# okgarces/deep-successor-features-for-transfer

Hardware: AMD Instinct MI355X
Metric: env steps/sec (whole node), Reacher 8-task SF-DQN at 1/2/4/8 MI355X (higher is better)
Workload: dtype fp32; 1 GPU; reacher17-all-T8-B32 (Reacher-shape |s|=17 |a|=7 d=8, psi MLP 256x2, all heads updated per env step: main_sfdqn_torch.py path); heads_per_gpu=8, heads_total=8, global_batch=32, replay=host, parallelism=single

## Files before the change

deep-successor-features-for-transfer_amd/csrc/sfx.hip:

```cpp
#include <hip/hip_ext.h>
#include <hip/hip_runtime.h>
#include <dlfcn.h>
#include <rccl/rccl.h>

#include <cmath>
#include <cstdio>
#include <cstdlib>
#include <cstring>
#include <algorithm>
#include <atomic>
#include <chrono>
#include <deque>
#include <map>
#include <random>
#include <string>
#include <functional>
#include <tuple>
#include <utility>
#include <vector>

#include "sfx_kernels.h"
#include "sfx_gpiw.h"
#include "sfx_tsf.h"
#include "sfx_phi.h"
// ... 512 lines not shown
  A.npol = npol;
  A.guess = guess;
  A.flag = flag;
  A.flag_value = h->T;
  A.next_stride = next_stride;
  A.a = a;
  A.phi = phi;
  A.gamma = gamma;
  A.next = next;
  A.prev = skip ? prev : nullptr;
  A.skip = skip ? h->skip : nullptr;
  A.skipc = skip ? h->skipc : nullptr;
  launch(h, K_TDG, by, k_tdg, dim3(M, npol), dim3(256), h->G, A);
  LAUNCHCHK();
  return SFX_OK;
}

struct TdgSpec {
  int use_gpi = 1, guess = R_S1, next_stride = 0;
  const int64_t* a = nullptr;
  const float* gamma = nullptr;
  int64_t* next = nullptr;
  int* flag = nullptr;
  const int* xmax = nullptr;
  int poloff = 0;
  const int* xi_src = nullptr;
  int* xi_dst = nullptr;
  int xi_copy = 0, xi_n = 0;
  const int64_t* prev = nullptr;
  bool skip = false;
  const float* dz_scale = nullptr;
};

int tdg_variant(const sfx_handle* h) {
  if ((h->d & 3) != 0 || h->O > TDG_ROWS_O || h->A > 128) return 0;
  const long ta = (long)h->T * h->A;
  if (h->d <= 8 && 32 * ta <= 256 * 8) return 1;
  if (h->d <= 16 && 32 * ta <= 256 * 4) return 2;
  return 0;
}

bool can_fuse_tdg(const sfx_handle* h) { return tdg_variant(h) != 0; }

struct BwdExtra {
  int inc_step = 1;
  bool fuse_v0 = false;
  int vRole = R_V;
  const float* v_x = nullptr;
  const float* v_xn = nullptr;
  bool skip_fwd = false;
  const float* ax = nullptr;
  int aM = 0, a_noskip = 0;
  bool* skip_armed = nullptr;
  std::function<bool(int li, int tail_at, const BwdArgs& A, int ntile, double bytes)> ride;
};

bool can_fuse_v0(const sfx_handle* h, int vM) { return h->L[0].K <= KFUSE && vM * h->L[0].K <= VFUSE; }
bool can_fuse_ahead(const sfx_handle* h, int vM, int aM) {
  const int K = h->L[0].K;
  return can_fuse_v0(h, vM) && ((vM * K + 3) & ~3) + 2 * aM * K <= VFUSE && (2 * aM * K) % 4 == 0;
}

int run_bwd(sfx_handle* h, int head0, int nhead, int M, const float* x0, const float* phi, const float* r,
            float* losses, const TdgSpec& td, const BwdExtra& ex = BwdExtra()) {
  const bool fuse = can_fuse_tdg(h) && ((uintptr_t)phi & 15) == 0 &&
                    (!td.xmax || 32 * h->A <= 1024);
  if (!fuse && td.xi_dst) SFX_FAIL(SFX_E_STATE, "run_bwd: maxima re-initialisation needs the fused TD launch");
  const bool armed = td.skip && (fuse ? M <= 32 : true);
  if (!fuse)
    RC(run_tdg(h, head0, nhead, td.guess, M, td.use_gpi, td.a, phi, td.gamma, td.next, td.next_stride, td.flag,
               td.xmax, td.poloff, td.dz_scale, td.prev, armed));
  if (ex.skip_armed) *ex.skip_armed = armed;
  const int tail_at = fuse ? 1 : 0;
  const bool need_tail = losses || r || !fuse;
  BwdArgs A{};
  A.M = M;
  A.head0 = head0;
  A.nhead = nhead;
  A.xcd = nhead > 1 ? 1 : 0;
  A.mask = h->mask;
  A.hp = h->hp_psi;
  A.hpw = h->hp_w;
  A.x0 = x0;
  A.phi = phi;
  A.r = r;
  A.train_w = r != nullptr;
  A.losses = losses;
  A.inc_step = ex.inc_step;
  A.step_in_tail = fuse ? 0 : 1;
  A.tdg_use_gpi = td.use_gpi;
  A.tdg_guess = td.guess;
  A.tdg_next_stride = td.next_stride;
  A.tdg_a = td.a;
  A.tdg_gamma = td.gamma;
  A.tdg_next = td.next;
  A.tdg_xmax = td.xmax;
  A.tdg_poloff = td.poloff;
  A.flag = td.flag;
  A.flag_value = h->T;
  A.dz_scale = td.dz_scale;
  A.xi_copy = td.xi_copy;
  A.xi_n = td.xi_n;
  A.dxs = 1;
  if (armed) {
    A.skip = h->skip;
    A.skip_v0 = ex.skip_fwd ? 1 : 0;
    if (fuse) {
      A.tdg_prev = td.prev;
      A.skipc = h->skipc;
    }
  }
  auto dw_tiles = [&](int l) { return cdiv(h->L[l].N, 32) * cdiv(h->L[l].K, 64); };
  auto geo = [&](int l) {
    const LayerGeo& L = h->L[l];
    const int xOff = l == 0 ? -1 : h->actOff[l - 1], dzIn = l == 0 ? 0 : h->actOff[l - 1];
    return RoleGeo{L.N, L.K, L.wOff, L.bOff, L.actIn, xOff,  h->actOff[l], dzIn};
  };
  auto dx_bytes = [&](int l) {
    const LayerGeo& L = h->L[l];
    return 4.0 * ((double)L.N * L.K + (double)M * L.N + 2.0 * M * L.K);
  };
  auto dw_bytes = [&](int l) {
    const LayerGeo& L = h->L[l];
    return 24.0 * ((double)L.N * L.K + L.N) + 4.0 * ((double)M * L.N + (double)M * L.K);
  };
  auto grid_of = [&](int ntile) { return A.xcd ? dim3(8 * cdiv(nhead, 8) * ntile) : dim3(ntile, nhead); };
  const bool merge = h->bwd_merge && nhead > 1 && !ex.ride && h->NL >= 3 && M <= 32 && ex.fuse_v0 &&
                     can_fuse_v0(h, M + (ex.v_xn ? 1 : 0)) && h->L[1].N <= DX_SPLIT_N;
  int l = h->NL - 1;
  if (fuse) {
    A.tdg = 1;
    A.xi_src = td.xi_src;
    A.xi_dst = td.xi_dst;
    A.ra = geo(l);
    const int ktiles = cdiv(h->L[l].K, 16);
    const bool rows16 = M > 16 && M <= 32 && h->tdg_rows != 32 &&
                        (h->tdg_rows == 16 || (nhead > 1 && !ex.ride && nhead * 2 * ktiles <= h->ncu));
    const int ntd = cdiv(M, rows16 ? 16 : 32) * ktiles;
    A.na = ntd;
    dim3 grid = grid_of(ntd);
    if (A.inc_step) A.adam_wg = (int)grid.x++ + 1;
    const double tdg_bytes = 4.0 * nhead * M * ((td.use_gpi ? h->T : 1) * h->O + 2.0 * h->O + 2.0 * h->d + 4);
    const bool v1 = tdg_variant(h) == 1;
    launch(h, K_BWD, nhead * dx_bytes(l) + tdg_bytes,
           rows16 ? (v1 ? k_bwd_tdg<2, 4, 16> : k_bwd_tdg<4, 2, 16>) : (v1 ? k_bwd_tdg<2, 8> : k_bwd_tdg<4, 4>), grid,
           dim3(256), h->G, A);
    A.adam_wg = 0;
    A.tdg = 0;
    A.xi_src = nullptr;
    A.xi_dst = nullptr;
    --l;
  }
  auto issue = [&](int li, bool mg, double by) {
    const int ntile = A.na + A.nb + A.nc + A.nd + A.tail;
    if (ex.ride && nhead == 1 && ex.ride(li, tail_at, A, ntile, by)) return;
    launch(h, K_BWD, by, !mg ? (h->bf16 ? k_bwd<true> : k_bwd<false>) : (h->bf16 ? k_bwd_mg<true> : k_bwd_mg<false>),
           grid_of(ntile), dim3(256), h->G, A);
  };
  for (; l >= (merge ? 2 : 1); --l) {
    const int li = h->NL - 1 - l;
    const bool dw = l < h->NL - 1;
    A.ra = geo(l);
    const bool split = h->dxpart && h->L[l].N > DX_SPLIT_N && M <= 32 * cdiv(h->Mmax, 32) && nhead <= h->T;
    A.dxs = split ? cdiv(h->L[l].N, DX_SPLIT_N) : 1;
    A.na = cdiv(M, 32) * cdiv(h->L[l].K, 16) * A.dxs;
    if (split) {
      A.dxpart = h->dxpart;
      A.dxctr = h->dxctr;
    }
    if (dw) {
      A.rb = geo(l + 1);
      A.nb = dw_tiles(l + 1);
    }
    A.tail = li == tail_at && need_tail ? 1 : 0;
    issue(li, false, nhead * (dx_bytes(l) + (dw ? dw_bytes(l + 1) : 0.0)));
  }
  const int last = merge ? h->NL - 2 : h->NL - 1;
  A.na = 0;
  A.dxs = 1;
  A.rb = geo(1);
  A.nb = dw_tiles(1);
  A.rc = geo(0);
  A.nc = dw_tiles(0);
  A.tail = last == tail_at && need_tail ? 1 : 0;
  double by_last = nhead * (dw_bytes(1) + dw_bytes(0));
  if (merge) {
    A.nc = cdiv(h->L[0].N, 16);
    A.ra = geo(1);
    A.rd = geo(2);
    A.nd = dw_tiles(2);
    by_last += nhead * (dw_bytes(2) + dx_bytes(1) - 4.0 * M * h->L[1].K - 4.0 * M * h->L[0].N);
  }
  A.vM = M + (ex.v_xn ? 1 : 0);
  A.vOff = h->actOff[0];
  A.vRole = ex.vRole;
  A.act0 = h->L[0].actOut;
  A.v_x = ex.v_x;
  A.v_xn = ex.v_xn;
  A.a_noskip = ex.a_noskip;
  if (ex.fuse_v0) {
    A.fuse_v0 = 1;
    A.ax = ex.ax;
    A.aM = ex.ax ? ex.aM : 0;
  }
  issue(last, merge, by_last);
  LAUNCHCHK();
  return SFX_OK;
}

GpiArgs gpi_args(int role, int rowoff, int row0, const float* w, float* psi, float* q, int64_t* task, int64_t* next,
                 int64_t* sel, int select_task, int use_gpi, int M) {
  GpiArgs A{};
  A.M = M;
  A.role = role;
  A.row0 = row0;
  A.rowoff = rowoff;
  A.select_task = select_task;
  A.use_gpi = use_gpi;
  A.w = w;
  A.psi_out = psi;
  A.q_out = q;
  A.task_out = task;
  A.next_out = next;
  A.sel_out = sel;
  return A;
}

int run_gpi(sfx_handle* h, const GpiArgs& A) {
  launch(h, K_GPI, 4.0 * A.M * ((double)h->T * h->O * (A.psi_out ? 2 : 1) + h->d + (A.q_out ? h->T * h->A : 0)),
         k_gpi, dim3(A.M), dim3(256), h->G, A);
  LAUNCHCHK();
  return SFX_OK;
}

int run_ver(sfx_handle* h, int M, int npol, bool sel, int post, const GpiArgs& g, const int64_t* spec,
            bool post_host = false) {
  VerArgs V{};
  V.M = M;
  V.post = post;
  V.npol = npol;
  V.sel = sel ? 1 : 0;
  V.spec_stride = MMAX;
  V.spec_next = spec;
  V.flag = &h->dout->flag;
  V.g = g;
  const int TA = h->T * h->A;
  V.rows = TA >= 256 ? 1 : (256 / TA < M ? 256 / TA : M);
  const bool wide = wide_gpi(h) && npol > 1;
  const dim3 grid = wide ? dim3(M, cdiv(npol, WPC) + 1) : dim3(npol + 1, cdiv(M, V.rows));
  if (sel && h->pub_res && h->fold_publish) {
    V.pub = h->pub_res;
    V.pub_dctr = h->pub_dctr;
    V.done = &h->dout->done;
    V.nblocks = (int)(grid.x * grid.y);
    h->pub_folded = true;
  } else if (post_host) {
    V.h_sel = h->hout->sel;
    V.h_flag = &h->hout->flag;
    V.h_posted = &h->hout->posted;
    V.done = &h->dout->done;
    V.nblocks = (int)(grid.x * grid.y);
    h->hout_posted = true;
  }
  const double by = 4.0 * (double)M * npol * h->T * h->O + 4.0 * h->T * h->O;
  if (wide)
    launch(h, K_VER, by, SFX_WIDE(k_verw), grid, dim3(256), h->G, V);
  else
    launch(h, K_VER, by, k_ver, grid, dim3(256), h->G, V);
  LAUNCHCHK();
  return SFX_OK;
}

void after_update(sfx_handle* h, int t) {
  h->host_step[t] += 1;
  h->since_target[t] += 1;
}

int maybe_sync_target(sfx_handle* h, int t) {
  if (h->since_target[t] >= h->target_update_ev) {
    touch(h);
    HIPCHK(hipMemcpyAsync(h->target_of(t), h->online_cur(t), sizeof(float) * h->P, hipMemcpyDeviceToDevice,
                          h->stream));
    if (h->bf16)
      HIPCHK(hipMemcpyAsync(h->tg16_of(t), h->on16_cur(t), sizeof(__bf16) * h->P, hipMemcpyDeviceToDevice,
                            h->stream));
    h->since_target[t] = 0;
  }
  return SFX_OK;
}

void pack_head(const sfx_handle* h, const float* src, float* dst) {
  std::memset(dst, 0, sizeof(float) * h->P);
  size_t off = 0;
  for (const LayerGeo& L : h->L) {
    std::memcpy(dst + L.wOff, src + off, sizeof(float) * L.N * L.K);
    off += (size_t)L.N * L.K;
    std::memcpy(dst + L.bOff, src + off, sizeof(float) * L.N);
    off += L.N;
  }
}

void unpack_head(const sfx_handle* h, const float* src, float* dst) {
  size_t off = 0;
  for (const LayerGeo& L : h->L) {
    std::memcpy(dst + off, src + L.wOff, sizeof(float) * L.N * L.K);
    off += (size_t)L.N * L.K;
    std::memcpy(dst + off, src + L.bOff, sizeof(float) * L.N);
    off += L.N;
  }
}

bool valid_head(const sfx_handle* h, int t) { return h && t >= 0 && t < h->T; }
bool valid_w(const sfx_handle* h, int t) { return h && t >= 0 && t < h->Tg; }

__global__ void k_to_bf16(const float* __restrict__ src, __bf16* __restrict__ dst, long long n) {
  for (long long i = (long long)blockIdx.x * blockDim.x + threadIdx.x; i < n; i += (long long)gridDim.x * blockDim.x)
    dst[i] = (__bf16)src[i];
}

int refresh_bf16(sfx_handle* h, const float* src, __bf16* dst, long long n) {
  touch(h);
  hipLaunchKernelGGL(k_to_bf16, dim3((unsigned)std::min<long long>(1024, (n + 255) / 256)), dim3(256), 0, h->stream, src,
                     dst, n);
  LAUNCHCHK();
  return SFX_OK;
}

void free_all(sfx_handle* h) {
  clear_graphs(h);
  for (auto& r : h->prof_recs) {
    (void)hipEventDestroy(r.a);
    (void)hipEventDestroy(r.b);
  }
  for (hipEvent_t e : h->prof_pool) (void)hipEventDestroy(e);
  for (void* p : {(void*)h->online, (void*)h->target, (void*)h->am, (void*)h->av, (void*)h->w, (void*)h->wm,
                  (void*)h->wv, (void*)h->step, (void*)h->dcancel, (void*)h->adamc, (void*)h->act, (void*)h->dz, (void*)h->rowloss, (void*)h->spec_next, (void*)h->skip, (void*)h->skipc,
                  (void*)h->dout, (void*)h->dxpart, (void*)h->dxctr, (void*)h->qh, (void*)h->selk})
    if (p) (void)hipFree(p);
  if (h->hout) (void)hipHostFree(h->hout);
  if (h->xin) (void)hipHostFree(h->xin);
  if (h->ev_step) (void)hipEventDestroy(h->ev_step);
  if (h->on16) (void)hipFree(h->on16);
  if (h->tg16) (void)hipFree(h->tg16);
  if (h->host_ar_buf) (void)hipHostFree(h->host_ar_buf);
  for (int* p : {h->tsx, h->tsz})
    if (p) (void)hipFree(p);
  for (int* p : {h->xb[0], h->xb[1]})
    if (p) (void)hipFree(p);
  if (h->comm_rounds) (void)rccl().CommDestroy(h->comm_rounds);
  if (h->comm && h->comm_owned) (void)rccl().CommDestroy(h->comm);
  if (h->dstall) (void)hipFree(h->dstall);
  if (h->cap) (void)hipStreamDestroy(h->cap);
}

int auto_spec_rounds(int T_glob) { return T_glob >= 16 ? 3 : 2; }

// ... 1167 lines not shown
```

deep-successor-features-for-transfer_amd/csrc/sfx_kernels.h:

```cpp
#pragma once
#include <hip/hip_runtime.h>
#include <stdint.h>

#include <type_traits>

namespace sfx {

typedef float floatx4 __attribute__((ext_vector_type(4)));

constexpr int NLMAX = 8;
constexpr int MT = 32;
constexpr int QMAX = 8192;
constexpr int OMAX = 4096;
constexpr int DMAX = 256;
constexpr int MMAX = 1024;
constexpr int KFUSE = 64;
constexpr int GEMV_N = 512;
constexpr int GEMV_M = 4;
constexpr int DX_SPLIT_N = 256;
constexpr int VFUSE = 4096;
constexpr int TQF = 4096;

enum { ACT_NONE = 0, ACT_RELU = 1, ACT_TANH = 2 };
enum { R_S = 0, R_S1T = 1, R_S1 = 2, R_G = 3, R_A = 4, R_V = 5, R_V2 = 6, R_NS = 7, R_NS1T = 8, R_NS1 = 9, NROLE = 10 };
// ... 823 lines not shown
    return z < huber ? __fmul_rn(__fmul_rn(0.5f, z), z) : __fmul_rn(huber, __fsub_rn(z, __fmul_rn(0.5f, huber)));
  }
  return __fmul_rn(x, x);
}

__device__ __forceinline__ void tdg_skip_report(int* skip, unsigned long long* skipc, int pol, int T, bool differs,
                                                bool have_prev, int nrep) {
  int* word = skip + T + pol;
  const int old = __hip_atomic_fetch_add(word, differs ? 0x10001 : 1, __ATOMIC_RELAXED, __HIP_MEMORY_SCOPE_AGENT);
  if ((old & 0xFFFF) == nrep - 1) {
    const bool any = (old >> 16) != 0 || differs;
    skip[pol] = any ? 0 : 1;
    if (skipc && have_prev) {
      atomicAdd(skipc, 1ull);
      if (!any) atomicAdd(skipc + 1, 1ull);
    }
    __hip_atomic_store(word, 0, __ATOMIC_RELAXED, __HIP_MEMORY_SCOPE_AGENT);
  }
}

struct TdgArgs {
  int M, use_gpi, pol0, npol, guess, next_stride, flag_value, pad_;
  const int64_t* a;
  const float* phi;
  const float* gamma;
  int64_t* next;
  int* flag;
  const int* xmax;
  int poloff, pad2_;
  const float* dz_scale;
  const int64_t* prev;
  int* skip;
  unsigned long long* skipc;
};

__global__ __launch_bounds__(256) void k_tdg(Geo G, TdgArgs A) {
  PROBE_T(pt0);
  const int b = blockIdx.x, pol = A.pol0 + blockIdx.y, tid = threadIdx.x;
  const int T = G.T, Aa = G.A, d = G.d, O = G.O, M = A.M, NLm = G.lastOff;
  __shared__ float s_w[DMAX];
  __shared__ float s_q[QMAX];
  __shared__ float s_t[OMAX];
  __shared__ float s_m[256];
  __shared__ float s_sq[DMAX];
  __shared__ int s_next;
  const float* wrow = G.w + (long long)pol * G.dpad;
  for (int k = tid; k < d; k += 256) s_w[k] = wrow[k];
  if (A.flag && b == 0 && blockIdx.y == 0 && tid == 0) *A.flag = A.flag_value;
  const float* trow = G.actp(R_S1T, pol, NLm) + (size_t)b * O;
  for (int o = tid; o < O; o += 256) s_t[o] = trow[o];
  const int ab = (int)A.a[b];
  const bool aok = ab >= 0 && ab < Aa;
  float cval = 0.f, phik = 0.f;
  const float gam = A.gamma[b];
  if (tid < d) {
    phik = A.phi[(size_t)b * d + tid];
    if (aok) cval = G.actp(R_S, pol, NLm)[(size_t)b * O + ab * d + tid];
  }
  __syncthreads();
  if (A.xmax) {
    const int* xr = A.xmax + ((size_t)(A.poloff + pol) * M + b) * Aa;
    for (int a = tid; a < Aa; a += 256) s_m[a] = unsortable(xr[a]);
  } else {
    const int t0 = A.use_gpi ? 0 : pol, nt = A.use_gpi ? T : 1;
    const FDiv fA = fdiv(Aa);
    for (int idx = tid; idx < nt * Aa; idx += 256) {
      const int tq = idx / fA, t = t0 + tq, a = idx - tq * Aa;
      const float* p = G.actp(t < pol ? A.guess : R_S1, t, NLm) + (size_t)b * O + a * d;
      float q = 0.f;
#pragma unroll 8
      for (int k = 0; k < d; ++k) q = __builtin_fmaf(p[k], s_w[k], q);
      s_q[idx] = q;
    }
    __syncthreads();
    for (int a = tid; a < Aa; a += 256) {
      float mx = s_q[a];
      for (int t = 1; t < nt; ++t) mx = fmaxf(mx, s_q[t * Aa + a]);
      s_m[a] = mx;
    }
  }
  __syncthreads();
  if (tid == 0) {
    int am = 0;
    float qm = s_m[0];
    for (int a = 1; a < Aa; ++a)
      if (s_m[a] > qm) {
        qm = s_m[a];
        am = a;
      }
    s_next = am;
    SFX_CHK(b < A.next_stride || !A.next, b, A.next_stride, 0);
    if (A.next) A.next[(size_t)blockIdx.y * A.next_stride + b] = am;
    if (A.skip)
      tdg_skip_report(A.skip, A.skipc, pol, T, !A.prev || A.prev[(size_t)blockIdx.y * A.next_stride + b] != am,
                      A.prev != nullptr, M);
  }
  __syncthreads();
  const float norm = td_norm(G, M, O, A.dz_scale);
  float* grow = G.dzp(pol, NLm) + (size_t)b * O;
  const float* crow = G.actp(R_S, pol, NLm) + (size_t)b * O;
  const int an = s_next;
  for (int o = tid; o < O; o += 256) {
    float gv = 0.f;
    if (aok && o >= ab * d && o < ab * d + d) {
      const int k = o - ab * d;
      const float tg = __fadd_rn(A.phi[(size_t)b * d + k], __fmul_rn(gam, s_t[an * d + k]));
      gv = td_grad(G.huber, norm, __fsub_rn(crow[o], tg));
    }
    grow[o] = gv;
  }
  float dsq = 0.f;
  if (tid < d && aok) {
    const float diff = __fsub_rn(cval, __fadd_rn(phik, __fmul_rn(gam, s_t[an * d + tid])));
    dsq = td_loss(G.huber, diff);
    if (!__builtin_isfinite(diff) && G.nonfin) atomicOr(G.nonfin, 1);
  }
  if (tid < d) s_sq[tid] = dsq;
  __syncthreads();
  if (tid == 0) {
    float s = 0.f;
    for (int k = 0; k < d; ++k) s = __fadd_rn(s, s_sq[k]);
    SFX_CHK(pol >= 0 && pol < G.T && b < MMAX, pol, b, 0);
    G.rowloss[(long long)pol * MMAX + b] = s;
  }
  PROBE_REC(17, pt0);
}

struct RoleGeo {
  int N, K, wOff, bOff, actIn;
  int xOff;
  int dzOff;
  int dzIn;
};

struct BwdArgs {
  int M, na, nb, nc, tail, head0, train_w, inc_step;
  int xcd, nhead;
  int step_in_tail;
  int tdg, tdg_use_gpi, tdg_guess, tdg_next_stride, flag_value;
  int adam_wg;
  const int64_t* tdg_a;
  const float* tdg_gamma;
  int64_t* tdg_next;
  const int* tdg_xmax;
  int tdg_poloff, pad3_;
  int* flag;
  int fuse_v0, vM, vOff, act0;
  int vRole, dxs;
  unsigned long long mask;
  float* dxpart;
  unsigned* dxctr;
  RoleGeo ra, rb, rc;
  RoleGeo rd;
  int nd, pad5_;
  AdamHP hp, hpw;
  const float* x0;
  const float* phi;
  const float* r;
  float* losses;
  const float* v_x;
  const float* v_xn;
  const float* ax;
  int aM, a_noskip;
  const int* xi_src;
  int* xi_dst;
  int xi_copy, xi_n;
  const int64_t* tdg_prev;
  int* skip;
  unsigned long long* skipc;
  int skip_v0;
  const float* dz_scale;
};
static_assert(sizeof(BwdArgs) == 512, "BwdArgs: the kernel-argument layout of k_bwd* / k_bwd_tsf");

__device__ __forceinline__ const float* layer_input(const Geo& G, const BwdArgs& A, int head, int xOff) {
  return xOff < 0 ? A.x0 : G.actp(R_S, head, xOff);
}

constexpr int TDG_ROWS_O = 128;
template <int RT>
struct TdgSmem {
  float w[32], gam[RT], ph[RT * 16];
  int a[RT], n[RT];
  float q[RT * 64], m[RT * 128];
  float tt[RT * TDG_ROWS_O], tc[RT * TDG_ROWS_O];
  float dz[RT * TDG_ROWS_O];
};

template <int VMAX, int U, int RT>
__device__ int tdg_rows(const Geo& G, const BwdArgs& A, int pol, int m0, bool pub, TdgSmem<RT>& sm) {
  static_assert(RT == 32 || RT == 16, "row tile of the fused TD launch");
  constexpr int U4 = RT / 8;
  const int tid = threadIdx.x, T = G.T, Aa = G.A, d = G.d, O = G.O, NLm = G.lastOff, M = A.M;
  const int nb = M - m0 < RT ? M - m0 : RT;
  const bool xm = A.tdg_xmax != nullptr;
  const int t0 = A.tdg_use_gpi ? 0 : pol, nt = A.tdg_use_gpi ? T : 1, TA = nt * Aa, n = xm ? 0 : nb * TA, V = d >> 2;
  const int guess = A.tdg_guess;
  const FDiv fTA = fdiv(TA), fA = fdiv(Aa);
  float4 v[U][VMAX];
#pragma unroll
  for (int u = 0; u < U; ++u) {
    const int idx = tid + u * 256;
    const bool ok = idx < n;
    const int bl = idx / fTA, rem = idx - bl * TA, tq = rem / fA, t = t0 + tq, a = rem - tq * Aa;
    const float4* p = reinterpret_cast<const float4*>(G.actp(t < pol ? guess : R_S1, ok ? t : 0, NLm) +
                                                      (ok ? (size_t)(m0 + bl) * O + a * d : 0));
#pragma unroll
    for (int j = 0; j < VMAX; ++j) v[u][j] = (ok && j < V) ? p[j] : make_float4(0.f, 0.f, 0.f, 0.f);
  }
  const int n4 = (nb * O) >> 2;
  const float4* tg4 = reinterpret_cast<const float4*>(G.actp(R_S1T, pol, NLm) + (size_t)m0 * O);
  const float4* cu4 = reinterpret_cast<const float4*>(G.actp(R_S, pol, NLm) + (size_t)m0 * O);
  float4 tt[U4], tc[U4];
#pragma unroll
  for (int u = 0; u < U4; ++u) {
    const int i = tid + u * 256;
    tt[u] = i < n4 ? tg4[i] : make_float4(0.f, 0.f, 0.f, 0.f);
    tc[u] = i < n4 ? cu4[i] : make_float4(0.f, 0.f, 0.f, 0.f);
  }
  const int np4 = (nb * d) >> 2;
  const float4 ph = tid < np4 ? reinterpret_cast<const float4*>(A.phi + (size_t)m0 * d)[tid] : make_float4(0.f, 0.f, 0.f, 0.f);
  const float wk = tid < d ? G.w[(long long)pol * G.dpad + tid] : 0.f;
  const int ab_l = tid < nb ? (int)A.tdg_a[m0 + tid] : 0;
  const float gam_l = tid < nb ? A.tdg_gamma[m0 + tid] : 0.f;
  int xv[U4];
  if (xm) {
    const int* xr = A.tdg_xmax + ((size_t)(A.tdg_poloff + pol) * M + m0) * Aa;
#pragma unroll
    for (int u = 0; u < U4; ++u) xv[u] = tid + u * 256 < nb * Aa ? xr[tid + u * 256] : 0;
  }
  const int64_t* prev = A.tdg_prev ? A.tdg_prev + (size_t)(pol - A.head0) * A.tdg_next_stride + m0 : nullptr;
  const int64_t prev_l = prev && tid < nb ? prev[tid] : -1;
#pragma unroll
  for (int u = 0; u < U4; ++u) {
    const int i = tid + u * 256;
    if (i < n4) {
      reinterpret_cast<float4*>(sm.tt)[i] = tt[u];
      reinterpret_cast<float4*>(sm.tc)[i] = tc[u];
      reinterpret_cast<float4*>(sm.dz)[i] = make_float4(0.f, 0.f, 0.f, 0.f);
    }
  }
  if (tid < np4) reinterpret_cast<float4*>(sm.ph)[tid] = ph;
  if (tid < d) sm.w[tid] = wk;
  if (tid < nb) {
    sm.a[tid] = ab_l;
    sm.gam[tid] = gam_l;
  }
  __syncthreads();
  PROBE_AT(3);
  if (xm) {
#pragma unroll
    for (int u = 0; u < U4; ++u)
      if (tid + u * 256 < nb * Aa) sm.m[tid + u * 256] = unsortable(xv[u]);
  }
#pragma unroll
  for (int u = 0; u < U; ++u) {
    const int idx = tid + u * 256;
    float q = 0.f;
#pragma unroll
    for (int j = 0; j < VMAX; ++j) {
      if (j < V) {
        q = __builtin_fmaf(v[u][j].x, sm.w[4 * j], q);
        q = __builtin_fmaf(v[u][j].y, sm.w[4 * j + 1], q);
        q = __builtin_fmaf(v[u][j].z, sm.w[4 * j + 2], q);
        q = __builtin_fmaf(v[u][j].w, sm.w[4 * j + 3], q);
      }
    }
    if (idx < n) sm.q[idx] = q;
  }
  __syncthreads();
  PROBE_AT(5);
  for (int i = tid; i < (xm ? 0 : nb * Aa); i += 256) {
    const int bl = i / fA, a = i - bl * Aa;
    const float* qb = sm.q + bl * TA + a;
    float mx = qb[0];
    for (int t = 1; t < nt; ++t) mx = fmaxf(mx, qb[t * Aa]);
    sm.m[i] = mx;
  }
  __syncthreads();
  PROBE_AT(6);
  const bool whole = m0 == 0 && nb == M;
  int differs = prev == nullptr;
  for (int bl = tid; bl < nb; bl += 256) {
    const float* mb = sm.m + bl * Aa;
    int am = 0;
    float qm = mb[0];
    for (int a = 1; a < Aa; ++a)
      if (mb[a] > qm) {
        qm = mb[a];
        am = a;
      }
    sm.n[bl] = am;
    if (prev && (bl == tid ? prev_l : prev[bl]) != am) differs = 1;
    SFX_CHK(!(pub && A.tdg_next) || (m0 + bl < A.tdg_next_stride && pol - A.head0 >= 0), pol, m0 + bl,
            A.tdg_next_stride);
    if (pub && A.tdg_next) A.tdg_next[(size_t)(pol - A.head0) * A.tdg_next_stride + m0 + bl] = am;
  }
  const int any = __syncthreads_or(differs);
  if (whole) {
    const int same = !any;
    if (pub && A.skip && tid == 0) {
      A.skip[pol] = same;
      if (A.skipc && prev) {
        atomicAdd(A.skipc, 1ull);
        if (same) atomicAdd(A.skipc + 1, 1ull);
      }
    }
// ... 127 lines not shown
  const int s = (threadIdx.x >> 6) & 1, Lx = threadIdx.x & 63, col = k0 + (Lx & 15);
  float xin[4] = {0.f, 0.f, 0.f, 0.f};
  if (threadIdx.x < NRED && col < K) {
#pragma unroll
    for (int i = 0; i < 4; ++i) {
      const int row = m0 + 16 * s + (Lx >> 4) * 4 + i;
      if (row < M) xin[i] = Xin[(size_t)row * K + col];
    }
  }
  floatx4 acc0 = {0.f, 0.f, 0.f, 0.f}, acc1 = {0.f, 0.f, 0.f, 0.f};
  if constexpr (TDG) {
    __shared__ TdgSmem<RT> sm;
    if (A.flag && tile == 0 && head == A.head0 && threadIdx.x == 0) *A.flag = A.flag_value;
    const int wpc = N > 64 ? 2 : 4, jw = 16 / wpc, j0 = (wave % wpc) * jw;
    const int nb = (wave / wpc) * 64 + g * 16;
    float bw[16];
#pragma unroll
    for (int j = 0; j < 16; ++j)
      bw[j] = (j >= j0 && j < j0 + jw && okk && nb + j < N) ? W[(size_t)(nb + j) * K + kk] : 0.f;
    if (tdg_rows<VMAX, U, RT>(G, A, head, m0, tile % ntk == 0, sm)) return;
    const float* da = sm.dz + (size_t)r * N + nb;
    const float* db = sm.dz + (size_t)(RT == 32 ? 16 + r : r) * N + nb;
#pragma unroll
    for (int j = 0; j < 16; ++j) {
      if (j >= j0 && j < j0 + jw) {
        const bool okj = nb + j < N;
        acc0 = mfma4(oka && okj ? da[j] : 0.f, bw[j], acc0);
        if constexpr (RT == 32) acc1 = mfma4(okb && okj ? db[j] : 0.f, bw[j], acc1);
      }
    }
  } else {
    const int kks[1] = {kk};
    floatx4 acc[1][2] = {{acc0, acc1}};
    dx_accum<BF, 1>(G.dzp(head, L.dzOff), W, BF ? G.on16 + G.slot_off(rslot(A.mask, head), head) + L.wOff : nullptr, N, K,
                    nbeg, nend, ma, mb, oka, okb, kks, acc);
    acc0 = acc[0][0];
    acc1 = acc[0][1];
  }
  PROBE_MARK();
  red[wave][0][lane] = acc0;
  if constexpr (RT == 32) red[wave][1][lane] = acc1;
  __syncthreads();
  if (!TDG && A.dxs > 1) {
    const int ntile = ((M + 31) >> 5) * ntk;
    const size_t pt = ((size_t)(head - A.head0) * ntile + tile) * A.dxs;
    __shared__ int s_last;
    if (threadIdx.x < 128) {
      const floatx4 v = dx_red_sum(red, s, Lx);
      float* o = A.dxpart + ((pt + split) * 128 + threadIdx.x) * 4;
#ifdef SFX_CHECK
      SFX_CHK((long long)((pt + split) * 128 + threadIdx.x) * 4 + 3 < G.ext_dxpart, pt, split, G.ext_dxpart);
#endif
#pragma unroll
      for (int i = 0; i < 4; ++i) st_coherent(o + i, v[i]);
      asm volatile("s_waitcnt vmcnt(0)" ::: "memory");
    }
    __syncthreads();
    if (threadIdx.x == 0) {
      unsigned* ctr = A.dxctr + (size_t)(head - A.head0) * ntile + tile;
      const unsigned prev = __hip_atomic_fetch_add(ctr, 1u, __ATOMIC_RELAXED, __HIP_MEMORY_SCOPE_AGENT);
      s_last = prev == (unsigned)A.dxs - 1;
      if (s_last) __hip_atomic_store(ctr, 0u, __ATOMIC_RELAXED, __HIP_MEMORY_SCOPE_AGENT);
    }
    __syncthreads();
    if (!s_last || threadIdx.x >= 128) return;
    floatx4 v = {0.f, 0.f, 0.f, 0.f};
    for (int q = 0; q < A.dxs; ++q) {
      const float* o = A.dxpart + ((pt + q) * 128 + threadIdx.x) * 4;
#pragma unroll
      for (int i = 0; i < 4; ++i) v[i] = __fadd_rn(v[i], ld_coherent(o + i));
    }
    if (col < K) {
#pragma unroll
      for (int i = 0; i < 4; ++i) {
        const int row = m0 + 16 * s + (Lx >> 4) * 4 + i;
        if (row < M) {
          G.chk_act(L.dzIn, (long long)row * K + col);
          out[(size_t)row * K + col] = act_bwd(v[i], xin[i], L.actIn);
        }
      }
    }
    return;
  }
  if (threadIdx.x < NRED) {
    const floatx4 v = dx_red_sum(red, s, Lx);
    if (col < K) {
#pragma unroll
      for (int i = 0; i < 4; ++i) {
        const int row = m0 + 16 * s + (Lx >> 4) * 4 + i;
        if (row < M) {
          G.chk_act(L.dzIn, (long long)row * K + col);
          out[(size_t)row * K + col] = act_bwd(v[i], xin[i], L.actIn);
        }
      }
    }
  }
}

__device__ __forceinline__ int v0_aoff(const BwdArgs& A, int K) { return (A.vM * K + 3) & ~3; }
constexpr int V0S = KFUSE + 4;

__device__ __forceinline__ void v0_tile(const float* x, int K, int m0, int rows, const float* w, float bb, int act,
                                        float* Y, int N, int n, long long lim) {
  constexpr int KS = 8;
  const int lane = threadIdx.x & 63, r = lane & 15, g = lane >> 4, ma = m0 + r;
  floatx4 c = {0.f, 0.f, 0.f, 0.f};
  for (int k0 = 0; k0 < K; k0 += 4 * KS) {
    float a[KS], b[KS];
#pragma unroll
    for (int q = 0; q < KS; ++q) {
      const int k = k0 + 4 * q + g;
      a[q] = (k < K && ma < rows) ? x[ma * K + k] : 0.f;
      b[q] = k < K ? w[k] : 0.f;
    }
#pragma unroll
    for (int q = 0; q < KS; ++q)
      if (k0 + 4 * q < K) c = mfma4(a[q], b[q], c);
  }
  if (n < N) {
#pragma unroll
    for (int i = 0; i < 4; ++i) {
      const int m = m0 + g * 4 + i;
      if (m < rows) {
        SFX_CHK((long long)m * N + n < lim, m, n, lim);
        Y[(size_t)m * N + n] = act_fwd(__fadd_rn(c[i], bb), act);
      }
    }
  }
}

template <int NW = 32>
__device__ __forceinline__ void fused_v0(const Geo& G, const BwdArgs& A, const RoleGeo& L, int head, int nbase, const float* sW,
                         const float* sB, const float* sX, const float* sWt = nullptr, const float* sBt = nullptr,
                         bool vrows = true, bool landed = false) {
  if (A.aM > 0 && !landed) asm volatile("s_waitcnt vmcnt(0)" ::: "memory");
  __syncthreads();
  PROBE_AT(3);
  const int K = L.K, N = L.N, VM = A.vM;
  static_assert(NW == 16 || NW == 32, "layer-0 tile width");
  constexpr int WS = NW == 32 ? 2 : 4;
  const int wave = threadIdx.x >> 6, lane = threadIdx.x & 63, r = lane & 15;
  const int wt = NW == 32 ? wave >> 1 : wave;
  const int nl = (NW == 32 ? (wave & 1) * 16 : 0) + r, n = nbase + nl;
  const float bias = sB[nl];
  if (vrows) {
    float* Y = G.actp(A.vRole, head, A.vOff);
    for (int mt = wt; mt * 16 < VM; mt += WS)
      v0_tile(sX, K, mt * 16, VM, sW + nl * V0S, bias, A.act0, Y, N, n, G.actSize - A.vOff);
  }
  PROBE_AT(4);
  if (A.aM > 0) {
    const int aM = A.aM, nt = (aM + 15) >> 4;
    const float* xa = sX + v0_aoff(A, K);
    const float bt = sBt[nl];
    for (int it = wt; it < 3 * nt; it += WS) {
      const int which = it / nt, mt = it - which * nt;
      v0_tile(xa + (which ? aM * K : 0), K, mt * 16, aM, which == 2 ? sWt + nl * K : sW + nl * V0S,
              which == 2 ? bt : bias, A.act0, G.actp(which == 0 ? R_NS : which == 1 ? R_NS1 : R_NS1T, head, A.vOff),
              N, n, G.actSize - A.vOff);
    }
  }
  PROBE_AT(5);
}

typedef __attribute__((address_space(3))) void* tsf_lds_t;

template <class F>
__device__ __forceinline__ void glds(float* dst, int n, F src, int w0 = 0, int nw = 4) {
  const int lane = threadIdx.x & 63, wv = (threadIdx.x >> 6) - w0;
  if (wv < 0 || wv >= nw) return;
  for (int c = wv; c * 64 < n; c += nw) {
    const int j = c * 64 + lane;
    const float* p = j < n ? src(j) : nullptr;
    if (p)
      __builtin_amdgcn_global_load_lds((const void*)p, (tsf_lds_t)(dst + c * 64), 4, 0, 0);
    else if (j < n)
      dst[j] = 0.f;
  }
}

template <int NW = 32>
struct V0Smem {
  float sW[NW * V0S];
  float sB[NW];
  float sWt[NW * KFUSE];
  float sBt[NW];
  __align__(16) float sX[VFUSE];
};
template <int NW = 32>
__device__ __forceinline__ V0Smem<NW>& v0_smem() {
  __shared__ V0Smem<NW> sm;
  return sm;
}

template <int NW>
__device__ __forceinline__ void v0_stage_ahead(const Geo& G, const BwdArgs& A, const RoleGeo& L, int head, int nbase,
                                               V0Smem<NW>& sm) {
  const int K = L.K, ncol = L.N - nbase < NW ? L.N - nbase : NW;
  const float* ax = A.ax;
  glds(sm.sX + v0_aoff(A, K), 2 * A.aM * K, [&](int j) -> const float* { return ax + j; });
  const float* Pt = G.target + (long long)head * G.P;
  const float* tw = Pt + L.wOff + (size_t)nbase * K;
  glds(sm.sWt, NW * K, [&](int j) -> const float* { return j < ncol * K ? tw + j : nullptr; });
  const float* tb = Pt + L.bOff + nbase;
  glds(sm.sBt, NW, [&](int j) -> const float* { return j < ncol ? tb + j : nullptr; }, 0, 1);
}

template <int NW = 32>
__device__ __forceinline__ void role_v0_only(const Geo& G, const BwdArgs& A, int head, const RoleGeo& L, int tile, bool vrows) {
  const int N = L.N, K = L.K, M = A.M, tid = threadIdx.x, nbase = tile * NW;
  const float* Pw = G.online + G.slot_off(rslot(A.mask, head) ^ 1, head);
  V0Smem<NW>& sm = v0_smem<NW>();
  float* sW = sm.sW;
  float* sB = sm.sB;
  float* sX = sm.sX;
  if (A.aM > 0) v0_stage_ahead(G, A, L, head, nbase, sm);
  const FDiv fK = fdiv(K);
  for (int j = tid; j < NW * K; j += 256) {
    const int nl = j / fK, k = j - nl * K;
    sW[nl * V0S + k] = nbase + nl < N ? Pw[L.wOff + (size_t)(nbase + nl) * K + k] : 0.f;
  }
  if (tid < NW) sB[tid] = nbase + tid < N ? Pw[L.bOff + nbase + tid] : 0.f;
  if (vrows) {
    const int nxs = A.vM * K;
    for (int j = tid; j < nxs; j += 256) sX[j] = j < M * K ? A.v_x[j] : A.v_xn[j - M * K];
  }
  fused_v0<NW>(G, A, L, head, nbase, sW, sB, sX, sm.sWt, sm.sBt, vrows);
}

template <bool BF = false, bool MG = false>
__device__ __forceinline__ void role_dw(const Geo& G, const BwdArgs& A, int head, const RoleGeo& L, int tile, bool fuse,
                                        floatx4 (*red)[2][64] = nullptr) {
  constexpr int NW = MG ? 16 : 32;
  constexpr int NH = MG ? 1 : 2;
  const int N = L.N, K = L.K, M = A.M;
  const int ntk = (K + 63) >> 6;
  const int kt = tile % ntk, nt = tile / ntk;
  const int wave = threadIdx.x >> 6, lane = threadIdx.x & 63, r = lane & 15, g = lane >> 4;
  const int nbase = nt * NW, n0 = MG ? nbase : nbase + (wave & 1) * 16;
  const int k0 = kt * 64 + (MG ? wave * 16 : (wave >> 1) * 32);
  const float* dZ = G.dzp(head, L.dzOff);
  const float* X = layer_input(G, A, head, L.xOff);
  const int rs = rslot(A.mask, head);
  const long long ro = G.slot_off(rs, head), wo = G.slot_off(rs ^ 1, head);
  const float* Pr = G.online + ro;
  const float* Mr = G.am + ro;
  const float* Vr = G.av + ro;
  float* Pw = G.online + wo;
  float* Mw = G.am + wo;
  float* Vw = G.av + wo;
  const AdamC c = G.adamc[head];
  const int cx = step_cancelled(G.cancel);
  const int nn = n0 + r, kb0 = k0 + r, kb1 = k0 + 16 + r;
  float pp[4 * NH], pm[4 * NH], pv[4 * NH];
  bool ok[4 * NH];
#pragma unroll
  for (int i = 0; i < 4; ++i) {
    const int n = n0 + g * 4 + i;
#pragma unroll
    for (int h = 0; h < NH; ++h) {
      const int k = h ? kb1 : kb0;
      const int e = i * NH + h;
      ok[e] = n < N && k < K;
      const size_t off = (size_t)L.wOff + (size_t)n * K + k;
      pp[e] = ok[e] ? Pr[off] : 0.f;
      pm[e] = ok[e] ? Mr[off] : 0.f;
      pv[e] = ok[e] ? Vr[off] : 0.f;
    }
  }
  const bool dob = kt == 0 && wave < (MG ? 1 : 2) && g == 0 && nn < N;
  const int nbias = nn;
  float bp = 0.f, bm = 0.f, bv = 0.f;
  if (dob) {
    bp = Pr[L.bOff + nbias];
    bm = Mr[L.bOff + nbias];
    bv = Vr[L.bOff + nbias];
  }
  constexpr int XQ = VFUSE / 1024;
  float4 xs[XQ];
  float xn = 0.f;
  const int nx = fuse ? M * K : 0;
  const int nxn = fuse && A.v_xn ? K : 0;
  if (fuse && A.aM > 0) v0_stage_ahead(G, A, L, head, nbase, v0_smem<NW>());
  if (fuse) {
    if ((nx & 3) == 0 && (reinterpret_cast<uintptr_t>(A.v_x) & 15) == 0) {
#pragma unroll
      for (int q = 0; q < XQ; ++q) {
        const int j = threadIdx.x + 256 * q;
        xs[q] = 4 * j < nx ? reinterpret_cast<const float4*>(A.v_x)[j] : make_float4(0.f, 0.f, 0.f, 0.f);
      }
    } else {
#pragma unroll
      for (int q = 0; q < XQ; ++q) {
        const int j = 4 * (threadIdx.x + 256 * q);
        xs[q].x = j < nx ? A.v_x[j] : 0.f;
        xs[q].y = j + 1 < nx ? A.v_x[j + 1] : 0.f;
        xs[q].z = j + 2 < nx ? A.v_x[j + 2] : 0.f;
        xs[q].w = j + 3 < nx ? A.v_x[j + 3] : 0.f;
      }
    }
    if ((int)threadIdx.x < nxn) xn = A.v_xn[threadIdx.x];
  }
  __builtin_amdgcn_sched_barrier(0);
  floatx4 acc0 = {0.f, 0.f, 0.f, 0.f}, acc1 = {0.f, 0.f, 0.f, 0.f};
  float bsum = 0.f;
  float dz0[MT / 4], xb0[MT / 4];
  if constexpr (MG) {
    static_assert(MT == 32, "merged tile: the 32 rows of one dX tile are the one row chunk of dW");
    const RoleGeo& L1 = A.ra;
    const float* Y0 = layer_input(G, A, head, L1.xOff);
    float y0[MT / 4];
#pragma unroll
    for (int j = 0; j < MT / 4; ++j) {
      const int m = 4 * j + g;
      y0[j] = (m < M && nn < N) ? Y0[(size_t)m * N + nn] : 0.f;
      xb0[j] = (m < M && kb0 < K) ? X[(size_t)m * K + kb0] : 0.f;
    }
    const int kks[1] = {nbase + r};
    floatx4 dacc[1][2] = {};
    dx_accum<BF, 1>(G.dzp(head, L1.dzOff), Pr + L1.wOff, BF ? G.on16 + ro + L1.wOff : nullptr, L1.N, L1.K, 0, L1.N, r,
                    16 + r, r < M, 16 + r < M, kks, dacc);
    red[wave][0][lane] = dacc[0][0];
    red[wave][1][lane] = dacc[0][1];
    PROBE_AT(6);
    __syncthreads();
#pragma unroll
    for (int j = 0; j < MT / 4; ++j) {
      const int s = j >> 2, Lx = (j & 3) * 16 + r;
      float v = red[0][s][Lx][g];
      v = __fadd_rn(v, red[1][s][Lx][g]);
      v = __fadd_rn(v, red[2][s][Lx][g]);
      v = __fadd_rn(v, red[3][s][Lx][g]);
      dz0[j] = (4 * j + g < M && nn < N) ? act_bwd(v, y0[j], L1.actIn) : 0.f;
    }
    PROBE_AT(7);
  }
  for (int mc = 0; mc < M; mc += MT) {
    float av[MT / 4], bv0[MT / 4], bv1[MT / 4];
#pragma unroll
    for (int j = 0; j < MT / 4; ++j) {
      const int m = mc + 4 * j + g;
      const bool okm = m < M;
      if constexpr (MG) {
        av[j] = dz0[j];
        bv0[j] = xb0[j];
        continue;
      }
      av[j] = (okm && nn < N) ? dZ[(size_t)m * N + nn] : 0.f;
      bv0[j] = (okm && kb0 < K) ? X[(size_t)m * K + kb0] : 0.f;
      bv1[j] = (okm && kb1 < K) ? X[(size_t)m * K + kb1] : 0.f;
    }
#pragma unroll
    for (int j = 0; j < MT / 4; ++j) {
      acc0 = mfma4(av[j], bv0[j], acc0);
      if constexpr (!MG) acc1 = mfma4(av[j], bv1[j], acc1);
    }
#pragma unroll
    for (int j = 0; j < MT / 4; ++j) bsum = __fadd_rn(bsum, av[j]);
  }
  bsum = __fadd_rn(bsum, __shfl_xor(bsum, 16));
  bsum = __fadd_rn(bsum, __shfl_xor(bsum, 32));
  if (fuse && A.aM > 0) asm volatile("s_waitcnt vmcnt(0)" ::: "memory");
  PROBE_MARK();
  V0Smem<NW>& sm = v0_smem<NW>();
  float* sW = sm.sW;
  float* sB = sm.sB;
  float* sX = sm.sX;
  if (fuse) {
#pragma unroll
    for (int q = 0; q < XQ; ++q) {
      const int j = threadIdx.x + 256 * q;
      if (4 * j + 3 < nx) {
        reinterpret_cast<float4*>(sX)[j] = xs[q];
      } else if (4 * j < nx) {
        sX[4 * j] = xs[q].x;
        if (4 * j + 1 < nx) sX[4 * j + 1] = xs[q].y;
        if (4 * j + 2 < nx) sX[4 * j + 2] = xs[q].z;
      }
    }
    if ((int)threadIdx.x < nxn) sX[nx + threadIdx.x] = xn;
  }
#pragma unroll
  for (int i = 0; i < 4; ++i) {
    const int n = n0 + g * 4 + i;
#pragma unroll
    for (int h = 0; h < NH; ++h) {
      const int e = i * NH + h;
      if (ok[e]) {
        const int k = h ? kb1 : kb0;
        const size_t off = (size_t)L.wOff + (size_t)n * K + k;
        SFX_CHK((long long)off < G.P, L.wOff, n, k);
        adam_apply(pp[e], pm[e], pv[e], h ? acc1[i] : acc0[i], c);
        if (!cx) {
          st_param(Pw + off, pp[e]);
          st_moment(Mw + off, pm[e]);
          st_moment(Vw + off, pv[e]);
          if constexpr (BF) G.on16[wo + off] = (__bf16)pp[e];
        }
        if (fuse) sW[(n - nbase) * V0S + k] = pp[e];
      }
    }
  }
  if (dob) {
    adam_apply(bp, bm, bv, bsum, c);
    if (!cx) {
      st_param(Pw + L.bOff + nbias, bp);
      st_moment(Mw + L.bOff + nbias, bm);
      st_moment(Vw + L.bOff + nbias, bv);
      if constexpr (BF) G.on16[wo + L.bOff + nbias] = (__bf16)bp;
    }
    if (fuse) sB[nbias - nbase] = bp;
  }
  if (fuse) fused_v0<NW>(G, A, L, head, nbase, sW, sB, sX, sm.sWt, sm.sBt, true, true);
}

__device__ __forceinline__ float block_sum(float v, float* red) {
  red[threadIdx.x] = v;
  __syncthreads();
#pragma unroll
  for (int s = 128; s >= 1; s >>= 1) {
    if ((int)threadIdx.x < s) red[threadIdx.x] = __fadd_rn(red[threadIdx.x], red[threadIdx.x + s]);
    __syncthreads();
  }
  const float r = red[0];
  __syncthreads();
  return r;
}

__device__ __forceinline__ void role_tail(const Geo& G, const BwdArgs& A, int head) {
  const int M = A.M, d = G.d, tid = threadIdx.x;
  __shared__ float s_e[MMAX];
  __shared__ float s_red[256];
  __shared__ float s_phi[2048];
  const int step = A.step_in_tail && A.inc_step ? G.step[head] + 1 : G.step[head];
  const int cx = step_cancelled(G.cancel);
  const float* rl = G.rowloss + (long long)head * MMAX;
  float* w = G.w + (long long)head * G.dpad;
  float part = 0.f;
  for (int b = tid; b < M; b += 256) part = __fadd_rn(part, rl[b]);
  float l2 = 0.f;
  if (A.train_w) {
    const bool lds_phi = M * d <= 2048;
    if (lds_phi)
      for (int j = tid; j < M * d; j += 256) s_phi[j] = A.phi[j];
    __syncthreads();
    const float* ph = lds_phi ? s_phi : A.phi;
    float se = 0.f;
    for (int b = tid; b < M; b += 256) {
      float rf = 0.f;
      for (int k = 0; k < d; ++k) rf = __builtin_fmaf(w[k], ph[(size_t)b * d + k], rf);
      s_e[b] = __fsub_rn(rf, A.r[b]);
      se = __builtin_fmaf(s_e[b], s_e[b], se);
    }
    se = block_sum(se, s_red);
    const AdamC c = adam_consts(A.hpw, step);
    const float nrm = (float)(2.0 / (double)M);
    float gw = 0.f;
    if (tid < d) {
      for (int b = 0; b < M; ++b) gw = __builtin_fmaf(__fmul_rn(nrm, s_e[b]), ph[(size_t)b * d + tid], gw);
    }
    __syncthreads();
    if (tid < d && !cx) adam_el(w + tid, G.wm + (long long)head * G.dpad + tid, G.wv + (long long)head * G.dpad + tid, gw, c);
    l2 = (float)((double)se / (double)M);
  }
  const float s = A.losses ? block_sum(part, s_red) : 0.f;
  if (tid == 0) {
    const float l1 = (float)((double)s / ((double)M * (double)G.O));
    if (A.losses) {
      float* lo = A.losses + 3 * (head - A.head0);
      lo[0] = __fadd_rn(l1, l2);
      lo[1] = l1;
      lo[2] = l2;
    }
    if (A.step_in_tail && !cx) {
      G.step[head] = step;
      G.adamc[head] = adam_consts(A.hp, step);
    }
  }
}

template <bool BF, bool MG = false>
__device__ __forceinline__ void bwd_body(const Geo& G, const BwdArgs& A, int head, int bx, floatx4 (*red)[2][64]) {
  PROBE_T(pt0);
  PROBE_MARKA();
  const bool skip = A.skip && __builtin_nontemporal_load(A.skip + head) != 0;
  if (bx < A.nc) {
    if (skip) {
      if (A.fuse_v0 && (!A.skip_v0 || (A.aM > 0 && A.a_noskip))) role_v0_only<MG ? 16 : 32>(G, A, head, A.rc, bx, !A.skip_v0);
      return;
    }
    role_dw<BF, MG>(G, A, head, A.rc, bx, A.fuse_v0 != 0, red);
    PROBE_REC(6, pt0);
    return;
  }
  bx -= A.nc;
  if (bx < A.nd) {
    if (skip) return;
    role_dw<BF>(G, A, head, A.rd, bx, false);
    PROBE_REC(5, pt0);
    return;
  }
  bx -= A.nd;
  if (bx < A.nb) {
    if (skip) return;
    role_dw<BF>(G, A, head, A.rb, bx, false);
    PROBE_REC(5, pt0);
    return;
  }
  bx -= A.nb;
  if (bx < A.na) {
    if (skip) return;
    role_dx<false, 2, 8, BF>(G, A, head, bx, red);
    PROBE_REC(4, pt0);
    return;
  }
  role_tail(G, A, head);
}

template <bool BF = false>
__global__ __launch_bounds__(256) void k_bwd(Geo G, BwdArgs A) {
  __shared__ floatx4 red[4][2][64];
  int head = A.head0 + blockIdx.y, bx = blockIdx.x;
  if (A.xcd) {
    if (!xcd_decode(blockIdx.x, A.nhead, A.na + A.nb + A.nc + A.nd + A.tail, head, bx)) return;
    head += A.head0;
  }
  bwd_body<BF>(G, A, head, bx, red);
}

template <bool BF = false>
__global__ __launch_bounds__(256) void k_bwd_mg(Geo G, BwdArgs A) {
  __shared__ floatx4 red[4][2][64];
  int head, bx;
  if (!xcd_decode(blockIdx.x, A.nhead, A.na + A.nb + A.nc + A.nd + A.tail, head, bx)) return;
  bwd_body<BF, true>(G, A, head + A.head0, bx, red);
}

template <int VMAX, int U, int RT = 32>
__global__ __launch_bounds__(256) void k_bwd_tdg(Geo G, BwdArgs A) {
  __shared__ floatx4 red[4][2][64];
  PROBE_T(pt0);
  if (A.xi_dst)
    fill_sortable(A.xi_dst, A.xi_src, A.xi_copy, A.xi_n, (blockIdx.y * gridDim.x + blockIdx.x) * 256 + threadIdx.x,
                  gridDim.x * gridDim.y * 256);
  if (A.adam_wg && (int)blockIdx.x == A.adam_wg - 1) {
    PROBE_MARKA();
    if (!step_cancelled(G.cancel)) {
      for (int i = threadIdx.x; i < A.nhead; i += 256) {
        const int hd = A.head0 + i, st = G.step[hd] + 1;
        const AdamC ac = adam_consts(A.hp, st);
        G.step[hd] = st;
        G.adamc[hd] = ac;
      }
    }
    PROBE_MARK();
    PROBE_REC(20, pt0);
    return;
  }
  int head = A.head0 + blockIdx.y, bx = blockIdx.x;
  if (A.xcd) {
    if (!xcd_decode(blockIdx.x, A.nhead, A.na, head, bx)) return;
    head += A.head0;
  }
  PROBE_MARKA();
  role_dx<true, VMAX, U, false, RT>(G, A, head, bx, red);
  PROBE_REC(3, pt0);
}

struct GpiArgs {
  int M, role, row0, select_task, use_gpi, rowoff;
  int w_stride, sel_stride;
  const float* w;
  float* psi_out;
  float* q_out;
  int64_t* task_out;
  int64_t* next_out;
  int64_t* sel_out;
  const unsigned long long* out_ind;
};

__device__ __forceinline__ unsigned long long argmax_key(float v, int idx) {
  const unsigned int u = __float_as_uint(__fadd_rn(v, 0.f));
  const unsigned int o = (u & 0x80000000u) ? ~u : (u | 0x80000000u);
  return ((unsigned long long)o << 32) | (unsigned long long)(0xFFFFFFFFu - (unsigned)idx);
}
__device__ __forceinline__ int argmax_idx(unsigned long long key) { return (int)(0xFFFFFFFFu - (unsigned)(key & 0xFFFFFFFFull)); }
__device__ __forceinline__ unsigned long long wave_max(unsigned long long k) {
#pragma unroll
  for (int m = 32; m >= 1; m >>= 1) {
    const unsigned long long o = __shfl_xor(k, m, 64);
    k = o > k ? o : k;
  }
  return k;
}

__device__ __forceinline__ int gpi_pick(const GpiArgs& A, const float* s_q, float* s_mt, float* s_ma, int T, int Aa,
                                        long long ob, int64_t* so, int nthr) {
  const int tid = threadIdx.x;
  for (int t = tid; t < T; t += nthr) {
    float mx = s_q[t * Aa];
    for (int a = 1; a < Aa; ++a) mx = fmaxf(mx, s_q[t * Aa + a]);
    s_mt[t] = mx;
  }
  for (int a = tid; a < Aa; a += nthr) {
    float mx = s_q[a];
    for (int t = 1; t < T; ++t) mx = fmaxf(mx, s_q[t * Aa + a]);
    s_ma[a] = mx;
  }
  __syncthreads();
  int picked = -1;
  if (tid < 64) {
    unsigned long long kt = 0ull, ka = 0ull;
    for (int t = tid; t < T; t += 64) {
      const unsigned long long k = argmax_key(s_mt[t], t);
      kt = k > kt ? k : kt;
    }
    for (int a = tid; a < Aa; a += 64) {
      const unsigned long long k = argmax_key(s_ma[a], a);
      ka = k > ka ? k : ka;
    }
    const int tb = argmax_idx(wave_max(kt)), ab = argmax_idx(wave_max(ka));
    const int c = A.use_gpi ? tb : A.select_task;
    unsigned long long kc = 0ull;
    if (so)
      for (int a = tid; a < Aa; a += 64) {
        const unsigned long long k = argmax_key(s_q[c * Aa + a], a);
        kc = k > kc ? k : kc;
      }
    const int act = so ? argmax_idx(wave_max(kc)) : 0;
    if (so) picked = c * Aa + act;
    if (tid == 0) {
      if (A.task_out) A.task_out[ob] = tb;
      if (A.next_out) A.next_out[ob] = ab;
      if (so) {
        __hip_atomic_store(so, (int64_t)c, __ATOMIC_RELAXED, __HIP_MEMORY_SCOPE_AGENT);
        __hip_atomic_store(so + 1, (int64_t)act, __ATOMIC_RELAXED, __HIP_MEMORY_SCOPE_AGENT);
      }
    }
  }
  return picked;
}

__device__ void gpi_row(const Geo& G, const GpiArgs& A0, int b) {
  GpiArgs A = A0;
  if (A.out_ind) {
    A.q_out = reinterpret_cast<float*>(A.out_ind[0]);
    A.task_out = reinterpret_cast<int64_t*>(A.out_ind[1]);
  }
  const int tid = threadIdx.x;
  const int T = G.T, Aa = G.A, d = G.d, O = G.O, NLm = G.lastOff, TA = T * Aa;
  __shared__ float s_q[QMAX];
  __shared__ float s_w[DMAX];
  __shared__ float s_mt[256], s_ma[256];
  const long long ob = (long long)(A.row0 + b);
  const int lb = A.rowoff + b;
  const FDiv fA = fdiv(Aa);
  const float* wr = A.w + ob * A.w_stride;
  int64_t* so = A.sel_out ? A.sel_out + ob * A.sel_stride : nullptr;
  if (A.psi_out) {
    const FDiv fO = fdiv(O);
    for (int idx = tid; idx < T * O; idx += 256) {
      const int t = idx / fO, o = idx - t * O;
      A.psi_out[(ob * T + t) * O + o] = G.actp(A.role, t, NLm)[(size_t)lb * O + o];
    }
  }
  if (TA <= 256 && (d & 3) == 0 && d <= 16 && ((uintptr_t)wr & 15) == 0) {
    const int V4 = d >> 2, t = tid / fA, a = tid - t * Aa;
    const bool act = tid < TA;
    const float4* p4 = reinterpret_cast<const float4*>(G.actp(A.role, act ? t : 0, NLm) + (size_t)lb * O + (act ? a * d : 0));
    const float4* w4 = reinterpret_cast<const float4*>(wr);
    float4 pv[4], wv[4];
#pragma unroll
    for (int j = 0; j < 4; ++j) {
      pv[j] = (act && j < V4) ? p4[j] : make_float4(0.f, 0.f, 0.f, 0.f);
      wv[j] = j < V4 ? w4[j] : make_float4(0.f, 0.f, 0.f, 0.f);
    }
    float q = 0.f;
#pragma unroll
    for (int j = 0; j < 4; ++j) {
      if (j < V4) {
        q = __builtin_fmaf(pv[j].x, wv[j].x, q);
        q = __builtin_fmaf(pv[j].y, wv[j].y, q);
        q = __builtin_fmaf(pv[j].z, wv[j].z, q);
        q = __builtin_fmaf(pv[j].w, wv[j].w, q);
      }
    }
    if (act) {
// ... 764 lines not shown
```

Baseline: 9256 env steps/s.

## Split target-network layer-0 recompute into extra workgroups in merged backward kernel

In the merged backward kernel, the layer-0 target-network forward (R_NS1T) that used to run inside the 16-wide fused v0 tiles now goes to separate dedicated workgroups appended to the grid. This happens only when the enlarged grid still fits within about three-eighths of the CUs. Those tiles then stage only the activations and skip loading the target weights. The merged path also stages v_x into LDS through asynchronous global-to-LDS loads instead of register staging. The aim is to shorten the critical path of the fused tiles, at the cost of more blocks and duplicated input staging.

```diff
diff --git a/deep-successor-features-for-transfer_amd/csrc/sfx.hip b/deep-successor-features-for-transfer_amd/csrc/sfx.hip
--- a/deep-successor-features-for-transfer_amd/csrc/sfx.hip
+++ b/deep-successor-features-for-transfer_amd/csrc/sfx.hip
@@ -688,7 +688,7 @@
     --l;
   }
   auto issue = [&](int li, bool mg, double by) {
-    const int ntile = A.na + A.nb + A.nc + A.nd + A.tail;
+    const int ntile = A.na + A.nb + A.nc + A.nd + A.tail + A.nt;
     if (ex.ride && nhead == 1 && ex.ride(li, tail_at, A, ntile, by)) return;
     launch(h, K_BWD, by, !mg ? (h->bf16 ? k_bwd<true> : k_bwd<false>) : (h->bf16 ? k_bwd_mg<true> : k_bwd_mg<false>),
            grid_of(ntile), dim3(256), h->G, A);
@@ -738,6 +738,10 @@
     A.fuse_v0 = 1;
     A.ax = ex.ax;
     A.aM = ex.ax ? ex.aM : 0;
+  }
+  if (merge && A.aM > 0) {
+    const int nt = cdiv(h->L[0].N, 16);
+    if (cdiv(nhead, 8) * (A.na + A.nb + A.nc + A.nd + A.tail + nt) <= h->ncu / 8 * 3) A.nt = nt;
   }
   issue(last, merge, by_last);
   LAUNCHCHK();
diff --git a/deep-successor-features-for-transfer_amd/csrc/sfx_kernels.h b/deep-successor-features-for-transfer_amd/csrc/sfx_kernels.h
--- a/deep-successor-features-for-transfer_amd/csrc/sfx_kernels.h
+++ b/deep-successor-features-for-transfer_amd/csrc/sfx_kernels.h
@@ -999,7 +999,7 @@
   unsigned* dxctr;
   RoleGeo ra, rb, rc;
   RoleGeo rd;
-  int nd, pad5_;
+  int nd, nt;
   AdamHP hp, hpw;
   const float* x0;
   const float* phi;
@@ -1433,8 +1433,10 @@
   if (A.aM > 0) {
     const int aM = A.aM, nt = (aM + 15) >> 4;
     const float* xa = sX + v0_aoff(A, K);
-    const float bt = sBt[nl];
-    for (int it = wt; it < 3 * nt; it += WS) {
+    int np = 3;
+    if constexpr (NW == 16) np = A.nt > 0 ? 2 : 3;
+    const float bt = np == 3 ? sBt[nl] : 0.f;
+    for (int it = wt; it < np * nt; it += WS) {
       const int which = it / nt, mt = it - which * nt;
       v0_tile(xa + (which ? aM * K : 0), K, mt * 16, aM, which == 2 ? sWt + nl * K : sW + nl * V0S,
               which == 2 ? bt : bias, A.act0, G.actp(which == 0 ? R_NS : which == 1 ? R_NS1 : R_NS1T, head, A.vOff),
@@ -1476,10 +1478,11 @@
 
 template <int NW>
 __device__ __forceinline__ void v0_stage_ahead(const Geo& G, const BwdArgs& A, const RoleGeo& L, int head, int nbase,
-                                               V0Smem<NW>& sm) {
+                                               V0Smem<NW>& sm, bool tgt = true) {
   const int K = L.K, ncol = L.N - nbase < NW ? L.N - nbase : NW;
   const float* ax = A.ax;
   glds(sm.sX + v0_aoff(A, K), 2 * A.aM * K, [&](int j) -> const float* { return ax + j; });
+  if (!tgt) return;
   const float* Pt = G.target + (long long)head * G.P;
   const float* tw = Pt + L.wOff + (size_t)nbase * K;
   glds(sm.sWt, NW * K, [&](int j) -> const float* { return j < ncol * K ? tw + j : nullptr; });
@@ -1495,7 +1498,7 @@
   float* sW = sm.sW;
   float* sB = sm.sB;
   float* sX = sm.sX;
-  if (A.aM > 0) v0_stage_ahead(G, A, L, head, nbase, sm);
+  if (A.aM > 0) v0_stage_ahead(G, A, L, head, nbase, sm, NW == 32 || A.nt == 0);
   const FDiv fK = fdiv(K);
   for (int j = tid; j < NW * K; j += 256) {
     const int nl = j / fK, k = j - nl * K;
@@ -1507,6 +1510,27 @@
     for (int j = tid; j < nxs; j += 256) sX[j] = j < M * K ? A.v_x[j] : A.v_xn[j - M * K];
   }
   fused_v0<NW>(G, A, L, head, nbase, sW, sB, sX, sm.sWt, sm.sBt, vrows);
+}
+
+__device__ __forceinline__ void role_v0_target(const Geo& G, const BwdArgs& A, int head, const RoleGeo& L, int tile) {
+  constexpr int NW = 16;
+  const int N = L.N, K = L.K, aM = A.aM, nbase = tile * NW, ncol = N - nbase < NW ? N - nbase : NW;
+  V0Smem<NW>& sm = v0_smem<NW>();
+  const float* x1 = A.ax + (size_t)aM * K;
+  glds(sm.sX, aM * K, [&](int j) -> const float* { return x1 + j; });
+  const float* Pt = G.target + (long long)head * G.P;
+  const float* tw = Pt + L.wOff + (size_t)nbase * K;
+  glds(sm.sWt, NW * K, [&](int j) -> const float* { return j < ncol * K ? tw + j : nullptr; });
+  const float* tb = Pt + L.bOff + nbase;
+  glds(sm.sBt, NW, [&](int j) -> const float* { return j < ncol ? tb + j : nullptr; }, 0, 1);
+  asm volatile("s_waitcnt vmcnt(0)" ::: "memory");
+  __syncthreads();
+  PROBE_MARK();
+  const int wave = threadIdx.x >> 6, nl = threadIdx.x & 15;
+  const float bt = sm.sBt[nl];
+  for (int mt = wave; mt * 16 < aM; mt += 4)
+    v0_tile(sm.sX, K, mt * 16, aM, sm.sWt + nl * K, bt, A.act0, G.actp(R_NS1T, head, A.vOff), N, nbase + nl,
+            G.actSize - A.vOff);
 }
 
 template <bool BF = false, bool MG = false>
@@ -1562,8 +1586,14 @@
   float xn = 0.f;
   const int nx = fuse ? M * K : 0;
   const int nxn = fuse && A.v_xn ? K : 0;
-  if (fuse && A.aM > 0) v0_stage_ahead(G, A, L, head, nbase, v0_smem<NW>());
-  if (fuse) {
+  if (fuse && A.aM > 0) v0_stage_ahead(G, A, L, head, nbase, v0_smem<NW>(), !MG || A.nt == 0);
+  if constexpr (MG) {
+    if (fuse) {
+      const float* vx = A.v_x;
+      const float* vxn = A.v_xn;
+      glds(v0_smem<NW>().sX, nx + nxn, [&](int j) -> const float* { return j < nx ? vx + j : vxn + (j - nx); });
+    }
+  } else if (fuse) {
     if ((nx & 3) == 0 && (reinterpret_cast<uintptr_t>(A.v_x) & 15) == 0) {
 #pragma unroll
       for (int q = 0; q < XQ; ++q) {
@@ -1641,13 +1671,13 @@
   }
   bsum = __fadd_rn(bsum, __shfl_xor(bsum, 16));
   bsum = __fadd_rn(bsum, __shfl_xor(bsum, 32));
-  if (fuse && A.aM > 0) asm volatile("s_waitcnt vmcnt(0)" ::: "memory");
+  if (fuse && (MG || A.aM > 0)) asm volatile("s_waitcnt vmcnt(0)" ::: "memory");
   PROBE_MARK();
   V0Smem<NW>& sm = v0_smem<NW>();
   float* sW = sm.sW;
   float* sB = sm.sB;
   float* sX = sm.sX;
-  if (fuse) {
+  if (!MG && fuse) {
 #pragma unroll
     for (int q = 0; q < XQ; ++q) {
       const int j = threadIdx.x + 256 * q;
@@ -1813,7 +1843,17 @@
 __global__ __launch_bounds__(256) void k_bwd_mg(Geo G, BwdArgs A) {
   __shared__ floatx4 red[4][2][64];
   int head, bx;
-  if (!xcd_decode(blockIdx.x, A.nhead, A.na + A.nb + A.nc + A.nd + A.tail, head, bx)) return;
+  const int nbody = A.na + A.nb + A.nc + A.nd + A.tail;
+  if (!xcd_decode(blockIdx.x, A.nhead, nbody + A.nt, head, bx)) return;
+  if (bx >= nbody) {
+    PROBE_T(pt0);
+    PROBE_MARKA();
+    const bool skip = A.skip && __builtin_nontemporal_load(A.skip + head + A.head0) != 0;
+    if (skip && A.skip_v0 && !A.a_noskip) return;
+    role_v0_target(G, A, head + A.head0, A.rc, bx - nbody);
+    PROBE_REC(21, pt0);
+    return;
+  }
   bwd_body<BF, true>(G, A, head + A.head0, bx, red);
 }
 
```

Result: slower. 8871 env steps/s (-4.2%).
